# vwxyzjn/cleanrl

Measured on AMD Instinct MI355X. Metric: env-steps/sec (SPS) PPO Breakout num_envs=1024 @1/2/4/8 MI355X; GAE HBM GB/s, higher is better.
Workload: dtype f32

## Files before the change

cleanrl_amd/build.py:

```python
from __future__ import annotations

import os
import subprocess
import sys
from concurrent.futures import ThreadPoolExecutor

CSRC = os.path.join(os.path.dirname(os.path.abspath(__file__)), "csrc")
LIB = os.path.join(CSRC, "libmi355ppo.so")
SOURCES = ["api.hip", "gae.hip", "distributions.hip", "loss.hip", "obs.hip", "optim.hip", "conv.hip", "convw.hip", "conv1q.hip", "conv1p.hip", "gemmz.hip", "gemmg.hip", "gemmh.hip", "convr.hip", "convrb.hip", "convrs.hip", "convrv.hip", "convu.hip", "fcw.hip", "heads.hip", "mlp.hip", "synth_env.hip", "dpcomm.hip", "lstm.hip", "trxl_attn.hip", "impala.hip", "pqn.hip", "pqn_lstm.hip", "offpolicy.hip", "sac.hip", "dqn.hip", "dqn_atari.hip", "rainbow.hip", "rainbow_twins.hip", "sac_atari.hip", "sac_atari_twins.hip", "qdagger.hip", "rnd.hip", "ppg.hip", "ppg_twins.hip", "ma_atari.hip", "ma_atari_twins.hip", "layernorm.hip", "layernorm_twins.hip", "host_twins.hip"]
HEADERS = ["common.h", "catrow.h", "ppo_rows.h", "lstm_rows.h", "trxl_rows.h", "impala_rows.h", "pqn_rows.h", "pqn_lstm_rows.h", "offpolicy_rows.h", "offpolicy_wg.h", "qhead_wg.h", "sac_rows.h", "dqn_rows.h", "dqn_atari_rows.h", "rainbow_rows.h", "sac_atari_rows.h", "qdagger_rows.h", "rnd_rows.h", "ppg_rows.h", "ma_atari_rows.h", "layernorm_rows.h", "conv1q_pack.h", "bf16split.h", "f16split.h", "conv_resident.h", "conv_resident_geom.h", "convr_geom.h", "convrb_geom.h", "convrs_geom.h", "convrv_geom.h", os.path.join("..", "..", "include", "mi355ppo.h")]
HIPCC = os.environ.get("HIPCC", "/opt/rocm/bin/hipcc")
FLAGS = ["--offload-arch=gfx950", "-O3", "-std=c++20", "-ffp-contract=off", "-fPIC", "-fvisibility=hidden", "-Wall", "-Wno-unused-function"]
EXTRA_FLAGS = {"conv.hip": ["-mllvm", "-pragma-unroll-threshold=1000000"], "gemmz.hip": ["-fno-slp-vectorize"], "gemmg.hip": ["-fno-slp-vectorize"], "gemmh.hip": ["-fno-slp-vectorize", "-mllvm", "-pragma-unroll-threshold=1000000"], "convr.hip": ["-fno-slp-vectorize", "-mllvm", "-pragma-unroll-threshold=1000000"], "convrb.hip": ["-fno-slp-vectorize", "-mllvm", "-pragma-unroll-threshold=1000000"], "convrs.hip": ["-fno-slp-vectorize", "-mllvm", "-pragma-unroll-threshold=1000000"], "convrv.hip": ["-fno-slp-vectorize", "-mllvm", "-pragma-unroll-threshold=1000000"], "convu.hip": ["-fno-slp-vectorize", "-mllvm", "-pragma-unroll-threshold=1000000"], "fcw.hip": ["-fno-slp-vectorize"], "convw.hip": ["-fno-slp-vectorize"], "lstm.hip": ["-fno-slp-vectorize"], "pqn_lstm.hip": ["-fno-slp-vectorize"]}


def _stale(target: str, deps: list[str]) -> bool:
    if not os.path.exists(target):
        return True
    t = os.path.getmtime(target)
    return any(os.path.getmtime(d) > t for d in deps)


def _run(cmd: list[str]) -> None:
    r = subprocess.run(cmd, cwd=CSRC, capture_output=True, text=True)
    if r.returncode != 0:
        raise RuntimeError("command failed: %s\n%s\n%s" % (" ".join(cmd), r.stdout, r.stderr))


def build(force: bool = False, verbose: bool = True) -> str:
    hdrs = [os.path.join(CSRC, h) for h in HEADERS]
    objs, jobs = [], []
    for src in SOURCES:
        obj = os.path.join(CSRC, src.replace(".hip", ".o"))
        objs.append(obj)
        if force or _stale(obj, [os.path.join(CSRC, src)] + hdrs):
            jobs.append([HIPCC] + FLAGS + EXTRA_FLAGS.get(src, []) + ["-c", src, "-o", obj])
    if jobs:
        if verbose:
            print(f"[cleanrl_amd.build] compiling {len(jobs)} HIP source(s) for gfx950", file=sys.stderr)
        with ThreadPoolExecutor(max_workers=min(len(jobs), os.cpu_count() or 1)) as ex:
            list(ex.map(_run, jobs))
    if force or jobs or _stale(LIB, objs):
        _run([HIPCC, "--offload-arch=gfx950", "-shared", "-o", LIB] + objs)
        if verbose:
            print(f"[cleanrl_amd.build] linked {LIB}", file=sys.stderr)
    return LIB


def build_tools(verbose: bool = True) -> str:
    root = os.path.dirname(os.path.dirname(CSRC))
    src = os.path.join(root, "tools", "conv_traffic.cpp")
    exe = os.path.join(root, "tools", "conv_traffic")
    if _stale(exe, [src, LIB, os.path.join(root, "include", "mi355ppo.h")]):
        _run([HIPCC, "--offload-arch=gfx950", "-O2", "-I" + os.path.join(root, "include"), src, "-o", exe, "-L" + CSRC,
              "-lmi355ppo", "-Wl,-rpath,$ORIGIN/../cleanrl_amd/csrc"])
        if verbose:
            print(f"[cleanrl_amd.build] built {exe}", file=sys.stderr)
    fsrc, fexe = os.path.join(root, "tools", "mfma_floor.cpp"), os.path.join(root, "tools", "mfma_floor")
    if os.path.exists(fsrc) and _stale(fexe, [fsrc]):
        _run([HIPCC, "--offload-arch=gfx950", "-O3", fsrc, "-o", fexe])
        if verbose:
            print(f"[cleanrl_amd.build] built {fexe}", file=sys.stderr)
    psrc, pexe = os.path.join(root, "tools", "hbm_probe.cpp"), os.path.join(root, "tools", "hbm_probe")
    if os.path.exists(psrc) and _stale(pexe, [psrc]):
        _run([HIPCC, "--offload-arch=gfx950", "-O3", psrc, "-o", pexe])
        if verbose:
            print(f"[cleanrl_amd.build] built {pexe}", file=sys.stderr)
    dsrc, dexe = os.path.join(root, "tools", "mfma_denorm.cpp"), os.path.join(root, "tools", "mfma_denorm")
    if os.path.exists(dsrc) and _stale(dexe, [dsrc]):
        _run([HIPCC, "--offload-arch=gfx950", "-O2", "-Wno-unused-result", dsrc, "-o", dexe])
        if verbose:
            print(f"[cleanrl_amd.build] built {dexe}", file=sys.stderr)
    return exe


if __name__ == "__main__":
    build(force="--force" in sys.argv)
    build_tools()
```

cleanrl_amd/csrc/common.h:

```cpp
#pragma once
#include <hip/hip_runtime.h>
#include <stdint.h>
#include <stdio.h>
#include <stdarg.h>
#include <stdlib.h>

#include "../../include/mi355ppo.h"

#define MI355_WAVE 64
#ifndef MI355_AUX_WGRAD_LD
#define MI355_AUX_WGRAD_LD 2
#endif
#ifndef MI355_AUX_STREAM_LD
#define MI355_AUX_STREAM_LD 0
#endif
#ifndef MI355_AUX_STREAM_ST
#define MI355_AUX_STREAM_ST 0
#endif
#define MI355_HD __host__ __device__ __forceinline__

namespace mi355ppo {

void set_error(const char* fmt, ...);

int conv1p_launch(const unsigned char* src, const int64_t* inds, const float* dz, float* part_w, float* part_b, int images, int grid,
                  hipStream_t s, const unsigned* dz_amax, float* partial_scale);
bool convw_applies(int64_t images, int layer, bool f16 = false);
int convw_parts(int64_t images, int layer);
int convw_launch(const float* src, const float* dz, float* part_w, float* part_b, int64_t images, int layer, int* nparts, hipStream_t s,
                 const unsigned* dz_amax = nullptr, const unsigned* src_amax = nullptr);

bool convr_on(long long images, long long min_images);
int convr_fwd3(const char* fn, const float* src, unsigned src_bytes, const void* pack, const float* bias, float* dst, unsigned dst_bytes, unsigned* bits,
               long long images, const unsigned* src_amax, unsigned* dst_amax, hipStream_t st);
int convr_fwd2(const char* fn, const float* src, unsigned src_bytes, const void* pack, const float* bias, float* dst, unsigned dst_bytes, unsigned* bits,
               long long images, const unsigned* src_amax, unsigned* dst_amax, hipStream_t st);
int convr_dgrad3(const char* fn, const float* dz, unsigned dz_bytes, const void* pack, const unsigned* bits, float* dsrc, unsigned dsrc_bytes,
                 long long images, const unsigned* dz_amax, unsigned* dsrc_amax, hipStream_t st);
int convr_dgrad2(const char* fn, const float* dz, unsigned dz_bytes, const void* pack, const unsigned* bits, float* dsrc, unsigned dsrc_bytes,
                 long long images, const unsigned* dz_amax, unsigned* dsrc_amax, hipStream_t st);
#ifndef MI355_RB_MIN_IMAGES
#define MI355_RB_MIN_IMAGES 3072
#endif
bool convrb_takes(long long images);
int convrb_dgrad2(const char* fn, const float* dz, unsigned dz_bytes, const void* pack, const unsigned* bits, float* dsrc, unsigned dsrc_bytes,
                  long long images, const unsigned* dz_amax, unsigned* dsrc_amax, hipStream_t st);
#ifndef MI355_RS_MIN_IMAGES
#define MI355_RS_MIN_IMAGES 512
#endif
bool convrs_takes(long long images);
int convrs_fwd2(const char* fn, const float* src, unsigned src_bytes, const void* pack, const float* bias, float* dst, unsigned dst_bytes, unsigned* bits,
                long long images, const unsigned* src_amax, unsigned* dst_amax, hipStream_t st);
#ifndef MI355_RV_MIN_IMAGES
#define MI355_RV_MIN_IMAGES 4096
#endif
bool convrv_takes(long long images);
int convrv_dgrad3(const char* fn, const float* dz, unsigned dz_bytes, const void* pack, const unsigned* bits, float* dsrc, unsigned dsrc_bytes,
                  long long images, const unsigned* dz_amax, unsigned* dsrc_amax, hipStream_t st);
int convu_max_parts();
bool convu_takes(int64_t images, int layer);
int convu_launch(const float* src, const float* dz, float* part_w, float* part_b, int64_t images, int layer, int* nparts, hipStream_t s,
                 const unsigned* dz_amax, const unsigned* src_amax);
int convu1_launch(const unsigned char* frames, const int64_t* inds, const float* dz, float* part_w, float* part_b, int64_t images, int* nparts,
                  hipStream_t s, const unsigned* dz_amax);
bool gemmg_on(long long rows, long long min_rows);
int gemmg_launch(const char* fn, int epi, const float* A, int lda, const void* pack, const float* bias, const unsigned* bits, float* C, int M, int N,
                 int K, const unsigned* a_amax, unsigned* c_amax, hipStream_t s);
bool gemmh_takes(int M, int N, int K, int lddz);
int gemmh_slabs();
int gemmh_launch(const float* dz, int lddz, const float* a, float* part, int M, int N, int K, const unsigned* dz_amax, const unsigned* a_amax, hipStream_t s);
int z_fc_raw_launch(const char* fn, const float* a, int lda, const void* pack, int M, int N, int K, void* ws, size_t ws_bytes, int* splits,
                    hipStream_t stream, const unsigned* a_amax = nullptr);

inline hipStream_t as_stream(void* s) { return reinterpret_cast<hipStream_t>(s); }

inline int bf16_term_pairs() {
    static const int n = [] {
        const char* e = getenv("MI355PPO_BF16_PAIRS");
        return (e && e[0] == '9') ? 9 : 6;
    }();
    return n;
}

inline bool kernel_switch(const char* name, long long size, long long default_min) {
    const char* e = getenv(name);
    if (!e || !e[0]) return size >= default_min;
    if (e[0] == '0' && !e[1]) return false;
    if (e[0] == 'm' && e[1] == 'i' && e[2] == 'n' && e[3] == ':') return size >= atoll(e + 4);
    return size >= default_min;
}

inline int cu_count() {
    int dev = 0, n = 0;
    if (hipGetDevice(&dev) != hipSuccess || hipDeviceGetAttribute(&n, hipDeviceAttributeMultiprocessorCount, dev) != hipSuccess || n <= 0) {
        (void)hipGetLastError();
        n = 256;
    }
    return n;
}

inline bool aligned(const void* p, size_t a) { return (reinterpret_cast<uintptr_t>(p) % a) == 0; }

inline int check_launch(const char* what) {
    hipError_t e = hipGetLastError();
    if (e != hipSuccess) {
        set_error("%s: %s", what, hipGetErrorString(e));
        return MI355PPO_EHIP;
    }
    return MI355PPO_OK;
}

#define MI355_REQUIRE(cond, code, ...)          \
    do {                                        \
        if (!(cond)) {                          \
            ::mi355ppo::set_error(__VA_ARGS__); \
            return (code);                      \
        }                                       \
    } while (0)

#ifdef __HIPCC__

MI355_HD uint32_t mulhi_u32(uint32_t a, uint32_t b) {
#if defined(__HIP_DEVICE_COMPILE__)
    return __umulhi(a, b);
#else
    return (uint32_t)(((uint64_t)a * (uint64_t)b) >> 32);
#endif
}

struct Philox {
    uint32_t k0, k1;
    MI355_HD Philox(uint64_t seed) : k0((uint32_t)seed), k1((uint32_t)(seed >> 32)) {}
    MI355_HD uint4 operator()(uint64_t ctr_lo, uint64_t ctr_hi) const {
        uint32_t c0 = (uint32_t)ctr_lo, c1 = (uint32_t)(ctr_lo >> 32), c2 = (uint32_t)ctr_hi, c3 = (uint32_t)(ctr_hi >> 32);
        uint32_t a = k0, b = k1;
#pragma unroll
        for (int r = 0; r < 10; ++r) {
            const uint32_t hi0 = mulhi_u32(0xD2511F53u, c0), lo0 = 0xD2511F53u * c0;
            const uint32_t hi1 = mulhi_u32(0xCD9E8D57u, c2), lo1 = 0xCD9E8D57u * c2;
            const uint32_t n0 = hi1 ^ c1 ^ a, n1 = lo1, n2 = hi0 ^ c3 ^ b, n3 = lo0;
            c0 = n0; c1 = n1; c2 = n2; c3 = n3;
            a += 0x9E3779B9u; b += 0xBB67AE85u;
        }
        return make_uint4(c0, c1, c2, c3);
    }
};

MI355_HD float u32_to_unit_open(uint32_t x) {
    return ((float)(x >> 9) + 0.5f) * (1.0f / 8388608.0f);
}


__device__ __forceinline__ float wave_sum(float v) {
#pragma unroll
    for (int off = 32; off > 0; off >>= 1) v += __shfl_xor(v, off, MI355_WAVE);
    return v;
}
__device__ __forceinline__ double wave_sum(double v) {
#pragma unroll
    for (int off = 32; off > 0; off >>= 1) v += __shfl_xor(v, off, MI355_WAVE);
    return v;
}

template <int NWAVES>
__device__ __forceinline__ double block_sum(double v, double* lds) {
    v = wave_sum(v);
    const int lane = threadIdx.x & 63, wave = threadIdx.x >> 6;
    if (lane == 0) lds[wave] = v;
    __syncthreads();
    double r = 0.0;
    if (threadIdx.x == 0) {
#pragma unroll
        for (int w = 0; w < NWAVES; ++w) r += lds[w];
    }
    __syncthreads();
    return r;
}

#endif
}
```

cleanrl_amd/csrc/convu.hip:

```cpp
#include "common.h"
#include "f16split.h"

#pragma clang fp contract(off)

namespace mi355ppo {

typedef float u_f32x16 __attribute__((ext_vector_type(16)));
typedef short u_s16x4 __attribute__((ext_vector_type(4)));
constexpr unsigned kUOob = 0xFFFFF000u;
constexpr int kURsrcWord3 = 0x00020000;

template <int SH_, int SW_, int C_, int KH_, int KW_, int S_, int OH_, int OW_, int LW_, int G_, int NW_, int OCC_>
struct UGeom {
    static constexpr int SH = SH_, SW = SW_, C = C_, KH = KH_, KW = KW_, S = S_, OH = OH_, OW = OW_, LW = LW_, G = G_, NW = NW_, OCC = OCC_, CO = 64;
    static constexpr int THREADS = 64 * NW, OP = OH * OW;
    static constexpr int PIXS = 4 * C + 16, LOS = 2 * C, PIXD = 4 * CO + 16, LOD = 2 * CO;
    static constexpr int SRC_REC = SH * SW;
    static constexpr int KPIX = LW > 0 ? G * OH * LW : (G * OP + 15) / 16 * 16, KSTEPS = KPIX / 16;
    static constexpr int SRC_SLACK = LW > 0 ? 3 : 0;
    static constexpr int SRCB = (G * SRC_REC + SRC_SLACK) * PIXS, DZB = KPIX * PIXD;
    static constexpr int UPS = C / 4, UPD = CO / 4;
    static constexpr int SRC_UNITS = G * SRC_REC * UPS, DZ_UNITS = G * OP * UPD;
    static constexpr int NIS = (SRC_UNITS + THREADS - 1) / THREADS, NID = (DZ_UNITS + THREADS - 1) / THREADS, NI = NIS + NID;
    static constexpr int PRE_PER = (NI + KSTEPS - 2) / (KSTEPS - 1);
    static constexpr int CT = C / 32, NTILES = KH * KW * CT, TPW = 2 * NTILES / NW;
    static constexpr int pidx(int y, int x) { return S == 2 ? y * SW + (x & 1) * (SW / 2) + (x >> 1) : y * SW + x; }
    static_assert(KPIX % 16 == 0 && 2 * NTILES % NW == 0 && THREADS % 16 == 0 && THREADS % UPS == 0 && SRCB + DZB <= 160 * 1024 && (S == 1 || SW % 2 == 0) && (LW == 0 || 16 % LW == 0), "shape");
};
using UGeom3 = UGeom<9, 9, 64, 3, 3, 1, 7, 7, 8, 4, 12, 3>;
using UGeom2 = UGeom<20, 20, 32, 4, 4, 2, 9, 9, 0, 2, 8, 2>;

template <class UG>
__global__ __launch_bounds__(UG::THREADS) __attribute__((amdgpu_waves_per_eu(UG::OCC, UG::OCC))) void convu_kernel(
    const float* __restrict__ src, const float* __restrict__ dz, float* __restrict__ part_w, float* __restrict__ part_b, long long images,
    int groups, unsigned src_bytes, unsigned dz_bytes, const unsigned* __restrict__ dz_amax, const unsigned* __restrict__ src_amax) {
    constexpr int NI = UG::NI, TPW = UG::TPW, PIXS = UG::PIXS, PIXD = UG::PIXD;
    __shared__ __attribute__((aligned(16))) unsigned char lds[UG::SRCB + UG::DZB];
    unsigned char* const lsrc = lds;
    unsigned char* const ldz = lds + UG::SRCB;
    const int tid = threadIdx.x, lane = tid & 63, wave = __builtin_amdgcn_readfirstlane(tid >> 6);
    const int g = lane >> 4, i = lane & 15, r = i >> 2, c4 = i & 3;
    const int ct = wave & 1, ng = wave >> 1;

    const int es = f16_scale_exp(amax_load(src_amax, lane)), ed = f16_scale_exp(amax_load(dz_amax, lane));
    const float ss = f16_pow2(es), sd = f16_pow2(ed), un = f16_unscale(es, ed);

    for (int o = tid * 16; o < UG::SRCB + UG::DZB; o += UG::THREADS * 16) *reinterpret_cast<s_u32x4*>(lds + o) = (s_u32x4){0u, 0u, 0u, 0u};

    const int half = g >> 1;
    const unsigned char* const dz_lane = ldz + (4 * r + 2 * half) * PIXD + (32 * ct + 16 * (g & 1) + 4 * c4) * 2;
    const int rline = r >> 1;
    const unsigned char* const src_lane = lsrc + (UG::LW > 0 ? (4 * (r & 1) + 2 * half) * PIXS : 0) + (16 * (g & 1) + 4 * c4) * 2;
    unsigned origin[UG::LW > 0 ? 1 : UG::KSTEPS];
    if constexpr (UG::LW == 0) {
#pragma unroll
        for (int s = 0; s < UG::KSTEPS; ++s) {
            unsigned pk = 0u;
#pragma unroll
            for (int t = 0; t < 2; ++t) {
                const int pix = 16 * s + 4 * r + 2 * half + t, gi = pix / UG::OP, p = pix - gi * UG::OP, y = p / UG::OW, x = p - y * UG::OW;
                const unsigned rec = pix < UG::G * UG::OP ? (unsigned)(gi * UG::SRC_REC + UG::pidx(UG::S * y, UG::S * x)) : 0u;
                pk |= rec << (16 * t);
            }
            origin[s] = pk;
        }
    }

    const __amdgpu_buffer_rsrc_t rsrc_s = __builtin_amdgcn_make_buffer_rsrc(const_cast<float*>(src), 0, (int)src_bytes, kURsrcWord3);
    const __amdgpu_buffer_rsrc_t rsrc_d = __builtin_amdgcn_make_buffer_rsrc(const_cast<float*>(dz), 0, (int)dz_bytes, kURsrcWord3);
    s_u32x4 pre[NI];
    float db4[4] = {0.0f, 0.0f, 0.0f, 0.0f};
    auto unit_dst = [&](int it) __attribute__((always_inline)) -> unsigned {
        if (it < UG::NIS) {
            const int u = it * UG::THREADS + tid, pix = u / UG::UPS, q4 = u - pix * UG::UPS, gi = pix / UG::SRC_REC, q = pix - gi * UG::SRC_REC, qy = q / UG::SW, qx = q - qy * UG::SW;
            return u < UG::SRC_UNITS ? (unsigned)((gi * UG::SRC_REC + UG::pidx(qy, qx)) * PIXS + q4 * 8) : ~0u;
        }
        const int v = (it - UG::NIS) * UG::THREADS + tid, q = v >> 4, gi = q / UG::OP, p = q - gi * UG::OP, y = p / UG::OW, x = p - y * UG::OW;
        const int rec = UG::LW > 0 ? (gi * UG::OH + y) * UG::LW + (((gi * UG::OH + y) & 1) ? x + 1 : x) : q;
        return v < UG::DZ_UNITS ? (unsigned)(UG::SRCB + rec * PIXD + (v & 15) * 8) : ~0u;
    };
    auto prefetch = [&](int grp, int it) __attribute__((always_inline)) {
        const bool any = grp < groups;
        if (it < UG::NIS) {
            const int u = it * UG::THREADS + tid;
            pre[it] = __builtin_bit_cast(s_u32x4, __builtin_amdgcn_raw_buffer_load_b128(rsrc_s, (any && u < UG::SRC_UNITS) ? (unsigned)grp * (unsigned)(UG::SRC_UNITS * 16) + (unsigned)u * 16u : kUOob, 0, MI355_AUX_WGRAD_LD));
        } else {
            const int v = (it - UG::NIS) * UG::THREADS + tid;
            pre[it] = __builtin_bit_cast(s_u32x4, __builtin_amdgcn_raw_buffer_load_b128(rsrc_d, (any && v < UG::DZ_UNITS) ? (unsigned)grp * (unsigned)(UG::DZ_UNITS * 16) + (unsigned)v * 16u : kUOob, 0, MI355_AUX_WGRAD_LD));
        }
    };
    auto fill = [&]() __attribute__((always_inline)) {
#pragma unroll
        for (int it = 0; it < NI; ++it) {
            const bool is_dz = it >= UG::NIS;
            unsigned hi[2], lo[2];
            f16_split4(pre[it], is_dz ? sd : ss, hi, lo);
            const unsigned d = unit_dst(it);
            if (d != ~0u) {
                *reinterpret_cast<uint2*>(lds + d) = make_uint2(hi[0], hi[1]);
                *reinterpret_cast<uint2*>(lds + d + (is_dz ? UG::LOD : UG::LOS)) = make_uint2(lo[0], lo[1]);
            }
            if (is_dz) {
#pragma unroll
                for (int c = 0; c < 4; ++c) db4[c] += __uint_as_float(pre[it][c]);
            }
        }
    };

    u_f32x16 acc[TPW];
#pragma unroll
    for (int t = 0; t < TPW; ++t)
#pragma unroll
        for (int e = 0; e < 16; ++e) acc[t][e] = 0.0f;
    typedef u_s16x4 __attribute__((address_space(3))) * lds_v4;
    auto tr2 = [&](const unsigned char* p0, const unsigned char* p1) __attribute__((always_inline)) -> s_u32x4 {
        const u_s16x4 a = __builtin_amdgcn_ds_read_tr16_b64_v4i16((lds_v4)(p0));
        const u_s16x4 b = __builtin_amdgcn_ds_read_tr16_b64_v4i16((lds_v4)(p1));
        const uint2 ua = __builtin_bit_cast(uint2, a), ub = __builtin_bit_cast(uint2, b);
        return (s_u32x4){ua.x, ua.y, ub.x, ub.y};
    };

    int grp = blockIdx.x;
#pragma unroll
    for (int it = 0; it < NI; ++it) prefetch(grp, it);
    for (; grp < groups; grp += gridDim.x) {
        __syncthreads();
        fill();
        __syncthreads();
        s_u32x4 afr[2][2], bfr[2][2];
        auto load_a = [&](int par, int s) __attribute__((always_inline)) {
            const unsigned char* const dline = dz_lane + 16 * s * PIXD;
            afr[par][0] = tr2(dline, dline + PIXD);
            afr[par][1] = tr2(dline + UG::LOD, dline + PIXD + UG::LOD);
        };
        auto load_b = [&](int par, int s, int t) __attribute__((always_inline)) {
            const unsigned char *s0, *s1;
            if constexpr (UG::LW > 0) {
                constexpr int OH = UG::OH;
                const int L0 = 2 * s, L1 = 2 * s + 1;
                const int rec0 = (L0 / OH) * UG::SRC_REC + (L0 % OH) * UG::SW, rec1 = (L1 / OH) * UG::SRC_REC + (L1 % OH) * UG::SW;
                s0 = src_lane + (rline ? rec1 - 1 : rec0) * PIXS;
                s1 = s0 + PIXS;
            } else {
                s0 = src_lane + (origin[s] & 0xffffu) * PIXS;
                s1 = src_lane + (origin[s] >> 16) * PIXS;
            }
            const int tile = ng * TPW + t, tap = tile / UG::CT, cpart = tile - tap * UG::CT;
            const int ty = tap / UG::KW, tx = tap - ty * UG::KW;
            const int off = UG::pidx(ty, tx) * PIXS + 64 * cpart;
            bfr[par][0] = tr2(s0 + off, s1 + off);
            bfr[par][1] = tr2(s0 + off + UG::LOS, s1 + off + UG::LOS);
        };
        load_a(0, 0);
        load_b(0, 0, 0);
#pragma unroll
        for (int q = 0; q < UG::KSTEPS * TPW; ++q) {
            const int s = q / TPW, t = q - s * TPW;
            if (t == 0 && s >= 1) {
#pragma unroll
                for (int u = 0; u < UG::PRE_PER; ++u)
                    if ((s - 1) * UG::PRE_PER + u < NI) prefetch(grp + gridDim.x, (s - 1) * UG::PRE_PER + u);
            }
            if (q + 1 < UG::KSTEPS * TPW) {
                const int s1 = (q + 1) / TPW, t1 = (q + 1) - s1 * TPW;
                if (t1 == 0) load_a(s1 & 1, s1);
                load_b((q + 1) & 1, s1, t1);
            }
            __builtin_amdgcn_sched_barrier(0);
            const s_u32x4 a_hi = afr[s & 1][0], a_lo = afr[s & 1][1], b_hi = bfr[q & 1][0], b_lo = bfr[q & 1][1];
            acc[t] = __builtin_amdgcn_mfma_f32_32x32x16_f16(__builtin_bit_cast(s_f16x8, a_hi), __builtin_bit_cast(s_f16x8, b_hi), acc[t], 0, 0, 0);
            acc[t] = __builtin_amdgcn_mfma_f32_32x32x16_f16(__builtin_bit_cast(s_f16x8, a_hi), __builtin_bit_cast(s_f16x8, b_lo), acc[t], 0, 0, 0);
            acc[t] = __builtin_amdgcn_mfma_f32_32x32x16_f16(__builtin_bit_cast(s_f16x8, a_lo), __builtin_bit_cast(s_f16x8, b_hi), acc[t], 0, 0, 0);
            __builtin_amdgcn_sched_barrier(0);
        }
    }

    constexpr int K = UG::KH * UG::KW * UG::C;
    float* const pw = part_w + (size_t)blockIdx.x * (UG::CO * K);
    const int li = lane & 31, lh = lane >> 5;
#pragma unroll
    for (int t = 0; t < TPW; ++t) {
        const int tile = ng * TPW + t, tap = tile / UG::CT, cpart = tile - tap * UG::CT;
#pragma unroll
        for (int e = 0; e < 16; ++e) {
            const int co = 32 * ct + (e & 3) + 8 * (e >> 2) + 4 * lh;
            pw[co * K + tap * UG::C + 32 * cpart + li] = acc[t][e] * un;
        }
    }
    __syncthreads();
    float* const red = reinterpret_cast<float*>(lds);
#pragma unroll
    for (int c = 0; c < 4; ++c) red[(tid >> 4) * 64 + 4 * (tid & 15) + c] = db4[c];
    __syncthreads();
    if (tid < UG::CO) {
        float sum = 0.0f;
        for (int k = 0; k < UG::THREADS / 16; ++k) sum += red[k * 64 + tid];
        part_b[(size_t)blockIdx.x * UG::CO + tid] = sum;
    }
}

template <int NW_>
struct UGeom1 {
    static constexpr int FH = 84, FW = 84, FC = 4, FWP = 90, OH = 20, OW = 20, CO = 32, NW = NW_, THREADS = 64 * NW, TPW = 8 / NW;
    static constexpr int SLOT = 8, FROW = FWP * SLOT, FB = FH * FROW;
    static constexpr int PIXD = 4 * CO + 16, LOD = 2 * CO, DZB = OH * OW * PIXD;
    static constexpr int F_UNITS = FH * FW * FC / 16, D_UNITS = OH * OW * CO / 4;
    static constexpr int NIF = (F_UNITS + THREADS - 1) / THREADS, NID = (D_UNITS + THREADS - 1) / THREADS, NI = NIF + NID;
    static constexpr int KSTEPS = (OH / 4) * (OW / 4);
    static_assert(OH % 4 == 0 && OW % 4 == 0 && THREADS % 8 == 0 && FW % 4 == 0 && NI <= KSTEPS - 1 && FB + DZB <= 160 * 1024, "shape");
};

template <class UG>
__global__ __launch_bounds__(UG::THREADS) __attribute__((amdgpu_waves_per_eu(UG::NW / 4, UG::NW / 4))) void convu1_kernel(
    const unsigned char* __restrict__ frames, const long long* __restrict__ inds, const float* __restrict__ dz, float* __restrict__ part_w,
    float* __restrict__ part_b, int images, unsigned dz_bytes, const unsigned* __restrict__ dz_amax) {
    constexpr int NI = UG::NI, PIXD = UG::PIXD;
    __shared__ __attribute__((aligned(16))) unsigned char lds[UG::FB + UG::DZB];
    unsigned char* const lfr = lds;
    unsigned char* const ldz = lds + UG::FB;
    const int tid = threadIdx.x, lane = tid & 63, wave = __builtin_amdgcn_readfirstlane(tid >> 6);
    const int g = lane >> 4, i = lane & 15, r = i >> 2, c4 = i & 3, half = g >> 1;

    const int ed = f16_scale_exp(amax_load(dz_amax, lane));
    const float sd = f16_pow2(ed), un = f16_pow2(24 - ed);

    for (int o = tid * 16; o < UG::FB + UG::DZB; o += UG::THREADS * 16) *reinterpret_cast<s_u32x4*>(lds + o) = (s_u32x4){0u, 0u, 0u, 0u};

    const unsigned char* const dz_lane = ldz + (r * UG::OW + 2 * half) * PIXD + (16 * (g & 1) + 4 * c4) * 2;
    const unsigned char* const fr_lane = lfr + (4 * r + wave * UG::TPW) * UG::FROW + 4 * (2 * half) * UG::SLOT + (16 * (g & 1) + 4 * c4) * 2;

    const __amdgpu_buffer_rsrc_t rsrc_d = __builtin_amdgcn_make_buffer_rsrc(const_cast<float*>(dz), 0, (int)dz_bytes, kURsrcWord3);
    s_u32x4 pre[NI];
    float db4[4] = {0.0f, 0.0f, 0.0f, 0.0f};
    auto prefetch = [&](int img, int it) __attribute__((always_inline)) {
        const bool any = img < images;
        if (it < UG::NIF) {
            const int u = it * UG::THREADS + tid;
            const long long row = any ? (inds ? inds[img] : (long long)img) : 0;
            const __amdgpu_buffer_rsrc_t rsrc_f = __builtin_amdgcn_make_buffer_rsrc(const_cast<unsigned char*>(frames) + row * (UG::FH * UG::FW * UG::FC), 0,
                                                                                 any ? UG::FH * UG::FW * UG::FC : 0, kURsrcWord3);
            pre[it] = __builtin_bit_cast(s_u32x4, __builtin_amdgcn_raw_buffer_load_b128(rsrc_f, u < UG::F_UNITS ? (unsigned)u * 16u : kUOob, 0, MI355_AUX_WGRAD_LD));
        } else {
            const int v = (it - UG::NIF) * UG::THREADS + tid;
            pre[it] = __builtin_bit_cast(s_u32x4, __builtin_amdgcn_raw_buffer_load_b128(rsrc_d, (any && v < UG::D_UNITS) ? (unsigned)img * (unsigned)(UG::D_UNITS * 16) + (unsigned)v * 16u : kUOob, 0, MI355_AUX_WGRAD_LD));
        }
    };
    auto fill = [&]() __attribute__((always_inline)) {
#pragma unroll
        for (int it = 0; it < NI; ++it) {
            if (it < UG::NIF) {
                const int u = it * UG::THREADS + tid, row = u / (UG::FW / 4), x4 = u - row * (UG::FW / 4);
                if (u < UG::F_UNITS) {
                    s_u32x4 lo4, hi4;
#pragma unroll
                    for (int p = 0; p < 2; ++p) {
                        const unsigned w0 = pre[it][2 * p], w1 = pre[it][2 * p + 1];
                        const s_u32x4 e = {(w0 & 0xffu) | ((w0 & 0xff00u) << 8), ((w0 >> 16) & 0xffu) | ((w0 >> 24) << 16),
                                           (w1 & 0xffu) | ((w1 & 0xff00u) << 8), ((w1 >> 16) & 0xffu) | ((w1 >> 24) << 16)};
                        if (p == 0) lo4 = e; else hi4 = e;
                    }
                    unsigned char* const d = lfr + row * UG::FROW + 4 * x4 * UG::SLOT;
                    *reinterpret_cast<s_u32x4*>(d) = lo4;
                    *reinterpret_cast<s_u32x4*>(d + 16) = hi4;
                }
            } else {
                const int v = (it - UG::NIF) * UG::THREADS + tid;
                unsigned hi[2], lo[2];
                f16_split4(pre[it], sd, hi, lo);
                if (v < UG::D_UNITS) {
                    unsigned char* const d = ldz + (v >> 3) * PIXD + (v & 7) * 8;
                    *reinterpret_cast<uint2*>(d) = make_uint2(hi[0], hi[1]);
                    *reinterpret_cast<uint2*>(d + UG::LOD) = make_uint2(lo[0], lo[1]);
                }
#pragma unroll
                for (int c = 0; c < 4; ++c) db4[c] += __uint_as_float(pre[it][c]);
            }
        }
    };

    u_f32x16 acc[UG::TPW];
#pragma unroll
    for (int t = 0; t < UG::TPW; ++t)
#pragma unroll
        for (int e = 0; e < 16; ++e) acc[t][e] = 0.0f;
    typedef u_s16x4 __attribute__((address_space(3))) * lds_v4;
    auto tr2 = [&](const unsigned char* p0, const unsigned char* p1) __attribute__((always_inline)) -> s_u32x4 {
        const u_s16x4 a = __builtin_amdgcn_ds_read_tr16_b64_v4i16((lds_v4)(p0));
        const u_s16x4 b = __builtin_amdgcn_ds_read_tr16_b64_v4i16((lds_v4)(p1));
        const uint2 ua = __builtin_bit_cast(uint2, a), ub = __builtin_bit_cast(uint2, b);
        return (s_u32x4){ua.x, ua.y, ub.x, ub.y};
    };

    int img = blockIdx.x;
#pragma unroll
    for (int it = 0; it < NI; ++it) prefetch(img, it);
    for (; img < images; img += gridDim.x) {
        __syncthreads();
        fill();
        __syncthreads();
        s_u32x4 fr[2][2 + UG::TPW];
        auto load_step = [&](int par, int s) __attribute__((always_inline)) {
            const int y0 = 4 * (s / (UG::OW / 4)), x0 = 4 * (s % (UG::OW / 4));
            const unsigned char* const d = dz_lane + (y0 * UG::OW + x0) * PIXD;
            const unsigned char* const f = fr_lane + 4 * y0 * UG::FROW + 4 * x0 * UG::SLOT;
            fr[par][0] = tr2(d, d + PIXD);
            fr[par][1] = tr2(d + UG::LOD, d + PIXD + UG::LOD);
#pragma unroll
            for (int t = 0; t < UG::TPW; ++t) fr[par][2 + t] = tr2(f + t * UG::FROW, f + t * UG::FROW + 4 * UG::SLOT);
        };
        load_step(0, 0);
#pragma unroll
        for (int s = 0; s < UG::KSTEPS; ++s) {
            if (s >= 1 && s <= NI) prefetch(img + gridDim.x, s - 1);
            if (s + 1 < UG::KSTEPS) load_step((s + 1) & 1, s + 1);
            __builtin_amdgcn_sched_barrier(0);
#pragma unroll
            for (int t = 0; t < UG::TPW; ++t) {
                acc[t] = __builtin_amdgcn_mfma_f32_32x32x16_f16(__builtin_bit_cast(s_f16x8, fr[s & 1][0]), __builtin_bit_cast(s_f16x8, fr[s & 1][2 + t]), acc[t], 0, 0, 0);
                acc[t] = __builtin_amdgcn_mfma_f32_32x32x16_f16(__builtin_bit_cast(s_f16x8, fr[s & 1][1]), __builtin_bit_cast(s_f16x8, fr[s & 1][2 + t]), acc[t], 0, 0, 0);
            }
            __builtin_amdgcn_sched_barrier(0);
        }
    }

    float* const pw = part_w + (size_t)blockIdx.x * (UG::CO * 256);
    const int li = lane & 31, lh = lane >> 5;
#pragma unroll
    for (int t = 0; t < UG::TPW; ++t)
#pragma unroll
        for (int e = 0; e < 16; ++e) pw[((e & 3) + 8 * (e >> 2) + 4 * lh) * 256 + (wave * UG::TPW + t) * 32 + li] = acc[t][e] * un;
    __syncthreads();
    float* const red = reinterpret_cast<float*>(lds);
#pragma unroll
    for (int c = 0; c < 4; ++c) red[(tid >> 3) * 32 + 4 * (tid & 7) + c] = db4[c];
    __syncthreads();
    if (tid < UG::CO) {
        float sum = 0.0f;
        for (int k = 0; k < UG::THREADS / 8; ++k) sum += red[k * 32 + tid];
        part_b[(size_t)blockIdx.x * UG::CO + tid] = sum;
    }
}

bool convu_on(int layer) {
    const char* e = getenv("MI355PPO_CONV_U");
    if (!e || !e[0] || (e[0] == '1' && !e[1])) return true;
    if (e[0] == '0' && !e[1]) return false;
    for (; *e; ++e)
        if (*e == '0' + layer) return true;
    return false;
}

int convu_max_parts() { return 256; }

bool convu_takes(int64_t images, int layer) {
    if (images <= 0) return false;
    if (layer == 1) return convu_on(1) && (long long)images * 20 * 20 * 32 * 4 < (1LL << 32) - 8192;
    if ((layer != 2 && layer != 3) || !convu_on(layer)) return false;
    return (long long)images * (layer == 3 ? 9 * 9 * 64 : 20 * 20 * 32) * 4 < (1LL << 32) - 8192;
}

template <class UG>
static int convu_launch_t(const float* src, const float* dz, float* part_w, float* part_b, int64_t images, int* nparts, hipStream_t s,
                          const unsigned* dz_amax, const unsigned* src_amax) {
    const long long srcb = (long long)images * UG::SRC_REC * UG::C * 4, dzb = (long long)images * UG::OP * UG::CO * 4;
    static int cus = 0;
    if (cus == 0) {
        int dev = 0, n = 0;
        if (hipGetDevice(&dev) != hipSuccess || hipDeviceGetAttribute(&n, hipDeviceAttributeMultiprocessorCount, dev) != hipSuccess || n <= 0) {
            (void)hipGetLastError();
            n = 256;
        }
        cus = n < convu_max_parts() ? n : convu_max_parts();
    }
    const int groups = (int)((images + UG::G - 1) / UG::G);
    const int grid = groups < cus ? groups : cus;
    hipLaunchKernelGGL((convu_kernel<UG>), dim3((unsigned)grid), dim3(UG::THREADS), 0, s, src, dz, part_w, part_b, (long long)images, groups,
                       (unsigned)srcb, (unsigned)dzb, dz_amax, src_amax);
    *nparts = grid;
    return 0;
}

int convu_launch(const float* src, const float* dz, float* part_w, float* part_b, int64_t images, int layer, int* nparts, hipStream_t s,
                 const unsigned* dz_amax, const unsigned* src_amax) {
    if (!dz_amax || !src_amax || !convu_takes(images, layer)) return 1;
    return layer == 3 ? convu_launch_t<UGeom3>(src, dz, part_w, part_b, images, nparts, s, dz_amax, src_amax)
                      : convu_launch_t<UGeom2>(src, dz, part_w, part_b, images, nparts, s, dz_amax, src_amax);
}

int convu1_launch(const unsigned char* frames, const int64_t* inds, const float* dz, float* part_w, float* part_b, int64_t images, int* nparts,
                  hipStream_t s, const unsigned* dz_amax) {
    if (!dz_amax || !convu_takes(images, 1)) return 1;
    const long long dzb = (long long)images * 20 * 20 * 32 * 4;
    static int cus = 0;
    if (cus == 0) {
        int dev = 0, n = 0;
        if (hipGetDevice(&dev) != hipSuccess || hipDeviceGetAttribute(&n, hipDeviceAttributeMultiprocessorCount, dev) != hipSuccess || n <= 0) {
            (void)hipGetLastError();
            n = 256;
        }
        cus = n < convu_max_parts() ? n : convu_max_parts();
    }
    const int grid = images < cus ? (int)images : cus;
    hipLaunchKernelGGL((convu1_kernel<UGeom1<8>>), dim3((unsigned)grid), dim3(512), 0, s, frames, reinterpret_cast<const long long*>(inds), dz, part_w, part_b,
                       (int)images, (unsigned)dzb, dz_amax);
    *nparts = grid;
    return 0;
}

}
```

Baseline: 1.351 million.

## Add software-pipelined persistent conv1 weight-gradient kernel with LDS ring buffers

```diff
diff --git a/cleanrl_amd/build.py b/cleanrl_amd/build.py
--- a/cleanrl_amd/build.py
+++ b/cleanrl_amd/build.py
@@ -8,7 +8,7 @@
 CSRC = os.path.join(os.path.dirname(os.path.abspath(__file__)), "csrc")
 LIB = os.path.join(CSRC, "libmi355ppo.so")
 SOURCES = ["api.hip", "gae.hip", "distributions.hip", "loss.hip", "obs.hip", "optim.hip", "conv.hip", "convw.hip", "conv1q.hip", "conv1p.hip", "gemmz.hip", "gemmg.hip", "gemmh.hip", "convr.hip", "convrb.hip", "convrs.hip", "convrv.hip", "convu.hip", "fcw.hip", "heads.hip", "mlp.hip", "synth_env.hip", "dpcomm.hip", "lstm.hip", "trxl_attn.hip", "impala.hip", "pqn.hip", "pqn_lstm.hip", "offpolicy.hip", "sac.hip", "dqn.hip", "dqn_atari.hip", "rainbow.hip", "rainbow_twins.hip", "sac_atari.hip", "sac_atari_twins.hip", "qdagger.hip", "rnd.hip", "ppg.hip", "ppg_twins.hip", "ma_atari.hip", "ma_atari_twins.hip", "layernorm.hip", "layernorm_twins.hip", "host_twins.hip"]
-HEADERS = ["common.h", "catrow.h", "ppo_rows.h", "lstm_rows.h", "trxl_rows.h", "impala_rows.h", "pqn_rows.h", "pqn_lstm_rows.h", "offpolicy_rows.h", "offpolicy_wg.h", "qhead_wg.h", "sac_rows.h", "dqn_rows.h", "dqn_atari_rows.h", "rainbow_rows.h", "sac_atari_rows.h", "qdagger_rows.h", "rnd_rows.h", "ppg_rows.h", "ma_atari_rows.h", "layernorm_rows.h", "conv1q_pack.h", "bf16split.h", "f16split.h", "conv_resident.h", "conv_resident_geom.h", "convr_geom.h", "convrb_geom.h", "convrs_geom.h", "convrv_geom.h", os.path.join("..", "..", "include", "mi355ppo.h")]
+HEADERS = ["common.h", "catrow.h", "ppo_rows.h", "lstm_rows.h", "trxl_rows.h", "impala_rows.h", "pqn_rows.h", "pqn_lstm_rows.h", "offpolicy_rows.h", "offpolicy_wg.h", "qhead_wg.h", "sac_rows.h", "dqn_rows.h", "dqn_atari_rows.h", "rainbow_rows.h", "sac_atari_rows.h", "qdagger_rows.h", "rnd_rows.h", "ppg_rows.h", "ma_atari_rows.h", "layernorm_rows.h", "conv1q_pack.h", "bf16split.h", "f16split.h", "conv_resident.h", "conv_resident_geom.h", "convr_geom.h", "convrb_geom.h", "convrs_geom.h", "convrv_geom.h", "convus_geom.h", os.path.join("..", "..", "include", "mi355ppo.h")]
 HIPCC = os.environ.get("HIPCC", "/opt/rocm/bin/hipcc")
 FLAGS = ["--offload-arch=gfx950", "-O3", "-std=c++20", "-ffp-contract=off", "-fPIC", "-fvisibility=hidden", "-Wall", "-Wno-unused-function"]
 EXTRA_FLAGS = {"conv.hip": ["-mllvm", "-pragma-unroll-threshold=1000000"], "gemmz.hip": ["-fno-slp-vectorize"], "gemmg.hip": ["-fno-slp-vectorize"], "gemmh.hip": ["-fno-slp-vectorize", "-mllvm", "-pragma-unroll-threshold=1000000"], "convr.hip": ["-fno-slp-vectorize", "-mllvm", "-pragma-unroll-threshold=1000000"], "convrb.hip": ["-fno-slp-vectorize", "-mllvm", "-pragma-unroll-threshold=1000000"], "convrs.hip": ["-fno-slp-vectorize", "-mllvm", "-pragma-unroll-threshold=1000000"], "convrv.hip": ["-fno-slp-vectorize", "-mllvm", "-pragma-unroll-threshold=1000000"], "convu.hip": ["-fno-slp-vectorize", "-mllvm", "-pragma-unroll-threshold=1000000"], "fcw.hip": ["-fno-slp-vectorize"], "convw.hip": ["-fno-slp-vectorize"], "lstm.hip": ["-fno-slp-vectorize"], "pqn_lstm.hip": ["-fno-slp-vectorize"]}
diff --git a/cleanrl_amd/csrc/common.h b/cleanrl_amd/csrc/common.h
--- a/cleanrl_amd/csrc/common.h
+++ b/cleanrl_amd/csrc/common.h
@@ -63,6 +63,10 @@
                  const unsigned* dz_amax, const unsigned* src_amax);
 int convu1_launch(const unsigned char* frames, const int64_t* inds, const float* dz, float* part_w, float* part_b, int64_t images, int* nparts,
                   hipStream_t s, const unsigned* dz_amax);
+#ifndef MI355_US_MIN_IMAGES
+#define MI355_US_MIN_IMAGES 1024
+#endif
+bool convus_takes(long long images);
 bool gemmg_on(long long rows, long long min_rows);
 int gemmg_launch(const char* fn, int epi, const float* A, int lda, const void* pack, const float* bias, const unsigned* bits, float* C, int M, int N,
                  int K, const unsigned* a_amax, unsigned* c_amax, hipStream_t s);
diff --git a/cleanrl_amd/csrc/convu.hip b/cleanrl_amd/csrc/convu.hip
--- a/cleanrl_amd/csrc/convu.hip
+++ b/cleanrl_amd/csrc/convu.hip
@@ -1,5 +1,6 @@
 #include "common.h"
 #include "f16split.h"
+#include "convus_geom.h"
 
 #pragma clang fp contract(off)
 
@@ -199,16 +200,6 @@
     }
 }
 
-template <int NW_>
-struct UGeom1 {
-    static constexpr int FH = 84, FW = 84, FC = 4, FWP = 90, OH = 20, OW = 20, CO = 32, NW = NW_, THREADS = 64 * NW, TPW = 8 / NW;
-    static constexpr int SLOT = 8, FROW = FWP * SLOT, FB = FH * FROW;
-    static constexpr int PIXD = 4 * CO + 16, LOD = 2 * CO, DZB = OH * OW * PIXD;
-    static constexpr int F_UNITS = FH * FW * FC / 16, D_UNITS = OH * OW * CO / 4;
-    static constexpr int NIF = (F_UNITS + THREADS - 1) / THREADS, NID = (D_UNITS + THREADS - 1) / THREADS, NI = NIF + NID;
-    static constexpr int KSTEPS = (OH / 4) * (OW / 4);
-    static_assert(OH % 4 == 0 && OW % 4 == 0 && THREADS % 8 == 0 && FW % 4 == 0 && NI <= KSTEPS - 1 && FB + DZB <= 160 * 1024, "shape");
-};
 
 template <class UG>
 __global__ __launch_bounds__(UG::THREADS) __attribute__((amdgpu_waves_per_eu(UG::NW / 4, UG::NW / 4))) void convu1_kernel(
@@ -341,6 +332,215 @@
     }
 }
 
+template <bool GATHER>
+__global__ __launch_bounds__(USGeom::THREADS) __attribute__((amdgpu_waves_per_eu(2, 2))) void convus_kernel(
+    const unsigned char* __restrict__ frames, const long long* __restrict__ inds, const float* __restrict__ dz, float* __restrict__ part_w,
+    float* __restrict__ part_b, int images, unsigned dz_bytes, const unsigned* __restrict__ dz_amax) {
+    using UG = USGeom;
+    constexpr int NIF = UG::NIF, NID = UG::NID, PIXD = UG::PIXD, THREADS = UG::THREADS;
+    typedef __attribute__((address_space(3))) unsigned char* lptr;
+    typedef __attribute__((address_space(3))) s_u32x4* lptr16;
+    typedef unsigned us_u32x2 __attribute__((ext_vector_type(2)));
+    typedef __attribute__((address_space(3))) us_u32x2* lptr8;
+    __shared__ __attribute__((aligned(256))) unsigned char lds[UG::LDSB];
+    const lptr l0 = (lptr)lds;
+    const int tid = threadIdx.x, lane = tid & 63, wave = __builtin_amdgcn_readfirstlane(tid >> 6);
+    const int g = lane >> 4, i = lane & 15, r = i >> 2, c4 = i & 3, half = g >> 1;
+    const int step = (int)gridDim.x;
+
+    const int ed = f16_scale_exp(amax_load(dz_amax, lane));
+    const float sd = f16_pow2(ed), un = f16_pow2(24 - ed);
+
+    for (int o = tid * 16; o < UG::LDSB; o += THREADS * 16) *(lptr16)(l0 + o) = (s_u32x4){0u, 0u, 0u, 0u};
+
+    const int dz_lane = UG::RING + UG::lane_dz(r, half, g & 1, c4);
+    const int fr_lane = UG::lane_fr(r, half, g & 1, c4, wave);
+
+    int fdst[NIF], ddst[NID], dseq[NID];
+#pragma unroll
+    for (int f = 0; f < NIF; ++f) fdst[f] = UG::funit_dst(f * THREADS + tid);
+#pragma unroll
+    for (int it = 0; it < NID; ++it) {
+        ddst[it] = UG::unit_dst(it * THREADS + tid);
+        dseq[it] = (UG::round_chunk(it, wave) + (UG::dz_round_next(it) ? UG::CHUNKS : 0)) % UG::NSLOT;
+    }
+    const __amdgpu_buffer_rsrc_t rsrc_d = __builtin_amdgcn_make_buffer_rsrc(const_cast<float*>(dz), 0, (int)dz_bytes, kURsrcWord3);
+    auto row_of = [&](int img) __attribute__((always_inline)) -> long long {
+        if constexpr (GATHER) return inds[img < images ? img : images - 1];
+        else return (long long)img;
+    };
+    const __amdgpu_buffer_rsrc_t rsrc_i = __builtin_amdgcn_make_buffer_rsrc(const_cast<long long*>(inds), 0, GATHER ? images * 8 : 0, kURsrcWord3);
+    us_u32x2 prow = {0u, 0u};
+    auto get_row = [&](int img) __attribute__((always_inline)) {
+        if constexpr (GATHER) prow = __builtin_bit_cast(us_u32x2, __builtin_amdgcn_raw_buffer_load_b64(rsrc_i, (unsigned)(img < images ? img : images - 1) * 8u, 0, 0));
+    };
+    auto take_row = [&](int img) __attribute__((always_inline)) -> long long {
+        if constexpr (GATHER)
+            return (long long)(((unsigned long long)(unsigned)__builtin_amdgcn_readfirstlane((int)prow[1]) << 32) | (unsigned)__builtin_amdgcn_readfirstlane((int)prow[0]));
+        else return (long long)img;
+    };
+    auto rsrc_f_at = [&](long long row, int img) __attribute__((always_inline)) {
+        return __builtin_amdgcn_make_buffer_rsrc(const_cast<unsigned char*>(frames) + row * (UG::FH * UG::FW * UG::FC), 0, img < images ? UG::FH * UG::FW * UG::FC : 0, kURsrcWord3);
+    };
+    auto rsrc_f_of = [&](int img) __attribute__((always_inline)) { return rsrc_f_at(row_of(img), img); };
+    s_u32x4 pf[NIF], pd[NID];
+    float db4[4] = {0.0f, 0.0f, 0.0f, 0.0f};
+    auto get_f = [&](const __amdgpu_buffer_rsrc_t rf, int f) __attribute__((always_inline)) {
+        const int u = f * THREADS + tid;
+        pf[f] = __builtin_bit_cast(s_u32x4, __builtin_amdgcn_raw_buffer_load_b128(rf, u < UG::F_UNITS ? (unsigned)u * 16u : kUOob, 0, MI355_AUX_WGRAD_LD));
+    };
+    auto get_d = [&](int img, int it) __attribute__((always_inline)) {
+        const int v = it * THREADS + tid;
+        pd[it] = __builtin_bit_cast(s_u32x4, __builtin_amdgcn_raw_buffer_load_b128(rsrc_d, (img < images && v < UG::D_UNITS) ? (unsigned)img * (unsigned)(UG::D_UNITS * 16) + (unsigned)v * 16u : kUOob, 0, MI355_AUX_WGRAD_LD));
+    };
+    auto put_f = [&](int fbuf, int f) __attribute__((always_inline)) {
+        if (f * THREADS + tid < UG::F_UNITS) {
+            s_u32x4 lo4, hi4;
+#pragma unroll
+            for (int p = 0; p < 2; ++p) {
+                const unsigned w0 = pf[f][2 * p], w1 = pf[f][2 * p + 1];
+                const s_u32x4 e = {(w0 & 0xffu) | ((w0 & 0xff00u) << 8), ((w0 >> 16) & 0xffu) | ((w0 >> 24) << 16),
+                                   (w1 & 0xffu) | ((w1 & 0xff00u) << 8), ((w1 >> 16) & 0xffu) | ((w1 >> 24) << 16)};
+                if (p == 0) lo4 = e; else hi4 = e;
+            }
+            const lptr d = l0 + (fbuf + fdst[f]);
+            *(lptr16)(d) = lo4;
+            *(lptr16)(d + 16) = hi4;
+        }
+    };
+    auto put_d = [&](int rot, int it) __attribute__((always_inline)) {
+        unsigned hi[2], lo[2];
+        f16_split4(pd[it], sd, hi, lo);
+        int sl = rot + dseq[it];
+        sl = sl >= UG::NSLOT ? sl - UG::NSLOT : sl;
+        if (it * THREADS + tid < UG::D_UNITS) {
+            const lptr d = l0 + (UG::RING + sl * UG::CHB + ddst[it]);
+            *(lptr8)(d) = (us_u32x2){hi[0], hi[1]};
+            *(lptr8)(d + UG::LOD) = (us_u32x2){lo[0], lo[1]};
+        }
+#pragma unroll
+        for (int c = 0; c < 4; ++c) {
+            db4[c] += __uint_as_float(pd[it][c]);
+            asm volatile("" : "+v"(db4[c]));
+        }
+    };
+
+    u_f32x16 acc;
+#pragma unroll
+    for (int e = 0; e < 16; ++e) acc[e] = 0.0f;
+    typedef u_s16x4 __attribute__((address_space(3))) * lds_v4;
+    auto tr2 = [&](lptr p0, lptr p1) __attribute__((always_inline)) -> s_u32x4 {
+        const u_s16x4 a = __builtin_amdgcn_ds_read_tr16_b64_v4i16((lds_v4)(p0));
+        const u_s16x4 b = __builtin_amdgcn_ds_read_tr16_b64_v4i16((lds_v4)(p1));
+        const uint2 ua = __builtin_bit_cast(uint2, a), ub = __builtin_bit_cast(uint2, b);
+        return (s_u32x4){ua.x, ua.y, ub.x, ub.y};
+    };
+    s_u32x4 fr[2][3];
+    auto load_step = [&](int par, int s, int slotb, int fbuf) __attribute__((always_inline)) {
+        const lptr d = l0 + (dz_lane + slotb) + UG::kstep_dz(s);
+        const lptr f = l0 + (fr_lane + fbuf) + UG::kstep_fr(s);
+        fr[par][0] = tr2(d, d + PIXD);
+        fr[par][1] = tr2(d + UG::LOD, d + PIXD + UG::LOD);
+        fr[par][2] = tr2(f, f + 4 * UG::SLOT);
+    };
+
+    int img = blockIdx.x, rot = 0, fcur = 0;
+    {
+        const __amdgpu_buffer_rsrc_t rf = rsrc_f_of(img), rf1 = rsrc_f_of(img + step);
+#pragma unroll
+        for (int f = 0; f < NIF; ++f) get_f(rf, f);
+#pragma unroll
+        for (int it = 0; it <= 2; ++it) get_d(img, it);
+        __syncthreads();
+#pragma unroll
+        for (int s = 2; s < UG::KSTEPS; ++s) {
+#pragma unroll
+            for (int it = 0; it < NID; ++it)
+                if (s == UG::dz_round_step(it)) {
+                    if (UG::dz_round_next(it)) put_d(1, it);
+                    __builtin_amdgcn_sched_barrier(0);
+                    get_d(UG::dz_round_next(it) ? img + step : img, it);
+                    __builtin_amdgcn_sched_barrier(0);
+                }
+#pragma unroll
+            for (int f = 0; f < NIF; ++f)
+                if (s == UG::fr_round_step(f)) {
+                    put_f(0, f);
+                    __builtin_amdgcn_sched_barrier(0);
+                    get_f(rf1, f);
+                    __builtin_amdgcn_sched_barrier(0);
+                }
+        }
+        __syncthreads();
+        load_step(0, 0, 0, 0);
+    }
+    long long row2 = row_of(img + 2 * step);
+    get_row(img + 3 * step);
+    for (; img < images; img += step) {
+        const __amdgpu_buffer_rsrc_t rf2 = rsrc_f_at(row2, img + 2 * step);
+        const int fnxt = UG::FBP - fcur;
+        int slotb[UG::NSLOT];
+#pragma unroll
+        for (int k = 0; k < UG::NSLOT; ++k) {
+            const int sl = rot + k;
+            slotb[k] = (sl >= UG::NSLOT ? sl - UG::NSLOT : sl) * UG::CHB;
+        }
+#pragma unroll
+        for (int s = 0; s < UG::KSTEPS; ++s) {
+            const int j = UG::kstep_chunk(s);
+            if (s == UG::barrier_step(j)) __syncthreads();
+            if (s + 1 < UG::KSTEPS) load_step((s + 1) & 1, s + 1, slotb[UG::kstep_chunk(s + 1) % UG::NSLOT], fcur);
+            else load_step((s + 1) & 1, 0, slotb[UG::CHUNKS % UG::NSLOT], fnxt);
+#pragma unroll
+            for (int it = 0; it < NID; ++it)
+                if (s == UG::dz_round_step(it)) {
+                    put_d(rot, it);
+                    __builtin_amdgcn_sched_barrier(0);
+                    get_d(img + (UG::dz_round_next(it) ? 2 : 1) * step, it);
+                }
+#pragma unroll
+            for (int f = 0; f < NIF; ++f)
+                if (s == UG::fr_round_step(f)) {
+                    put_f(fnxt, f);
+                    __builtin_amdgcn_sched_barrier(0);
+                    get_f(rf2, f);
+                }
+            if (s == UG::KSTEPS - 1) {
+                row2 = take_row(img + 3 * step);
+                __builtin_amdgcn_sched_barrier(0);
+                get_row(img + 4 * step);
+            }
+            __builtin_amdgcn_sched_barrier(0);
+            acc = __builtin_amdgcn_mfma_f32_32x32x16_f16(__builtin_bit_cast(s_f16x8, fr[s & 1][0]), __builtin_bit_cast(s_f16x8, fr[s & 1][2]), acc, 0, 0, 0);
+            acc = __builtin_amdgcn_mfma_f32_32x32x16_f16(__builtin_bit_cast(s_f16x8, fr[s & 1][1]), __builtin_bit_cast(s_f16x8, fr[s & 1][2]), acc, 0, 0, 0);
+            __builtin_amdgcn_sched_barrier(0);
+        }
+        static_assert(UG::KSTEPS % 2 == 1, "k-step 0 of the next image was read into parity 1");
+#pragma unroll
+        for (int k = 0; k < 3; ++k) fr[0][k] = fr[1][k];
+        rot = rot + UG::CHUNKS % UG::NSLOT;
+        rot = rot >= UG::NSLOT ? rot - UG::NSLOT : rot;
+        fcur = fnxt;
+    }
+
+    float* const pw = part_w + (size_t)blockIdx.x * (UG::CO * 256);
+    const int li = lane & 31, lh = lane >> 5;
+#pragma unroll
+    for (int e = 0; e < 16; ++e) pw[((e & 3) + 8 * (e >> 2) + 4 * lh) * 256 + wave * 32 + li] = acc[e] * un;
+    __syncthreads();
+    float* const red = reinterpret_cast<float*>(lds);
+#pragma unroll
+    for (int c = 0; c < 4; ++c) red[(tid >> 3) * 32 + 4 * (tid & 7) + c] = db4[c];
+    __syncthreads();
+    if (tid < UG::CO) {
+        float sum = 0.0f;
+        for (int k = 0; k < THREADS / 8; ++k) sum += red[k * 32 + tid];
+        part_b[(size_t)blockIdx.x * UG::CO + tid] = sum;
+    }
+}
+
+bool convus_takes(long long images) { return kernel_switch("MI355PPO_CONV_US", images, MI355_US_MIN_IMAGES); }
+
 bool convu_on(int layer) {
     const char* e = getenv("MI355PPO_CONV_U");
     if (!e || !e[0] || (e[0] == '1' && !e[1])) return true;
@@ -401,8 +601,12 @@
         cus = n < convu_max_parts() ? n : convu_max_parts();
     }
     const int grid = images < cus ? (int)images : cus;
-    hipLaunchKernelGGL((convu1_kernel<UGeom1<8>>), dim3((unsigned)grid), dim3(512), 0, s, frames, reinterpret_cast<const long long*>(inds), dz, part_w, part_b,
-                       (int)images, (unsigned)dzb, dz_amax);
+    if (convus_takes(images))
+        hipLaunchKernelGGL(inds ? convus_kernel<true> : convus_kernel<false>, dim3((unsigned)grid), dim3(USGeom::THREADS), 0, s, frames, reinterpret_cast<const long long*>(inds), dz, part_w, part_b,
+                           (int)images, (unsigned)dzb, dz_amax);
+    else
+        hipLaunchKernelGGL((convu1_kernel<UGeom1<8>>), dim3((unsigned)grid), dim3(512), 0, s, frames, reinterpret_cast<const long long*>(inds), dz, part_w, part_b,
+                           (int)images, (unsigned)dzb, dz_amax);
     *nparts = grid;
     return 0;
 }
diff --git a/cleanrl_amd/csrc/convus_geom.h b/cleanrl_amd/csrc/convus_geom.h
--- /dev/null
+++ b/cleanrl_amd/csrc/convus_geom.h
@@ -0,0 +1,41 @@
+#pragma once
+
+namespace mi355ppo {
+
+template <int NW_>
+struct UGeom1 {
+    static constexpr int FH = 84, FW = 84, FC = 4, FWP = 90, OH = 20, OW = 20, CO = 32, NW = NW_, THREADS = 64 * NW, TPW = 8 / NW;
+    static constexpr int SLOT = 8, FROW = FWP * SLOT, FB = FH * FROW;
+    static constexpr int PIXD = 4 * CO + 16, LOD = 2 * CO, DZB = OH * OW * PIXD;
+    static constexpr int F_UNITS = FH * FW * FC / 16, D_UNITS = OH * OW * CO / 4;
+    static constexpr int NIF = (F_UNITS + THREADS - 1) / THREADS, NID = (D_UNITS + THREADS - 1) / THREADS, NI = NIF + NID;
+    static constexpr int KSTEPS = (OH / 4) * (OW / 4);
+    static_assert(OH % 4 == 0 && OW % 4 == 0 && THREADS % 8 == 0 && FW % 4 == 0 && NI <= KSTEPS - 1 && FB + DZB <= 160 * 1024, "shape");
+};
+
+struct USGeom : UGeom1<8> {
+    using U = UGeom1<8>;
+    static constexpr int PCOLS = OW / 4, CHUNKS = OH / 4, CSTEPS = PCOLS;
+    static constexpr int CREC = 4 * OW, CHB = CREC * PIXD, CUNITS = CREC * (CO / 4);
+    static constexpr int NSLOT = 3;
+    static constexpr int FBP = (FB + 255) / 256 * 256;
+    static constexpr int FSPARE = FBP - FB;
+    static constexpr int RING = 2 * FBP, LDSB = RING + NSLOT * CHB;
+    static constexpr int kstep_chunk(int s) { return s / CSTEPS; }
+    static constexpr int kstep_dz(int s) { return 4 * (s % CSTEPS) * PIXD; }
+    static constexpr int kstep_fr(int s) { return 16 * (s / PCOLS) * FROW + 16 * (s % PCOLS) * SLOT; }
+    static constexpr int lane_dz(int r, int half, int g1, int c4) { return (r * OW + 2 * half) * PIXD + (16 * g1 + 4 * c4) * 2; }
+    static constexpr int lane_fr(int r, int half, int g1, int c4, int ty) { return (4 * r + ty) * FROW + 8 * half * SLOT + (16 * g1 + 4 * c4) * 2; }
+    static constexpr int slot(int n) { return n % NSLOT; }
+    static constexpr int unit_chunk(int v) { return (v >> 3) / CREC; }
+    static constexpr int unit_dst(int v) { return ((v >> 3) % CREC) * PIXD + (v & 7) * 8; }
+    static constexpr int round_chunk(int it, int wave) { return (it * (THREADS / 8) + 8 * wave) / CREC; }
+    static constexpr int funit_dst(int u) { return (u / (FW / 4)) * FROW + (u % (FW / 4)) * 4 * SLOT; }
+    static constexpr bool dz_round_next(int it) { return it < 2; }
+    static constexpr int dz_round_step(int it) { return it == 0 ? 20 : it == 1 ? 22 : it == 2 ? 1 : it == 3 ? 6 : it == 4 ? 10 : it == 5 ? 12 : 15; }
+    static constexpr int fr_round_step(int f) { return f == 0 ? 3 : f == 1 ? 8 : f == 2 ? 13 : 17; }
+    static constexpr int barrier_step(int j) { return CSTEPS * j + CSTEPS - 1; }
+    static_assert(NID == 7 && NIF == 4 && KSTEPS == CHUNKS * CSTEPS && CHB % 256 == 0 && FBP % 256 == 0 && RING % 256 == 0 && LDSB <= 160 * 1024 && CREC % 8 == 0, "shape");
+};
+
+}
```

After: 1.354 million (median of 6 runs). No clear change (+0.2%).
